# AnamarijaKic/bioinfo1

Hardware: AMD Instinct MI355X
Metric: GCUPS (DP cell updates/s) at 1/2/4/8 GPUs; bit-exact score+CIGAR (higher is better)
Workload: dtype int32 semantics; packed int16 arithmetic where range-proven (fits_int16), else int32; 1 GPU; config 2: 10000 uniform 1000x1000 pairs per GPU, local, scoring 1,-1,-1, CIGAR on; pairs_per_gpu=10000, qlen=1000, tlen=1000, mode=local, cigar=True, cells_per_gpu=10000000000, cells_total=10000000000, parallelism=pairs range-split over 1 GPU(s)

## Files before the change

bioinfo1_amd/csrc/ta_api.hip:

```cpp
#include <hip/hip_runtime.h>
#include <rocprofiler-sdk-roctx/roctx.h>

#include <algorithm>
#include <cstdio>
#include <cstdlib>
#include <cstring>
#include <mutex>
#include <string>
#include <vector>

#include "../../include/team_align_c.h"
#include "ta_context.h"
#include "ta_host_batch.h"
#include "ta_internal.h"
#include "ta_pipeline_internal.h"
#include "ta_plan_driver.h"
#include "ta_planner.h"

using ta_host::fail;

struct TA_PLAN_LOCAL ta_plan : ta::PlanArrays {
    ta_context* ctx = nullptr;
    ta::Plan h;
    void* own_block = nullptr;
    static int exec_chunk(ta_plan* pl, const ta_device_io* io, hipStream_t s, uint32_t c, bool fill, ta::TraceParts trace);
    uint32_t code_layout() const { return h.blk ? (h.ck ? 2u : 1u) : 0u; }
    uint32_t* err_word() const { return h.flexes.empty() && h.duals.empty() && h.single_tasks.empty() ? nullptr : d_err; }
    static const char* err_message(uint32_t err) {
        if (err & ta::kErrWalkCap) return "traceback: a band walk reached its event cap with cost left; results of this plan are invalid";
        return "packed fill: a pass hand-off poll timed out; results of this plan are invalid";
    }
};

namespace {

int check_args(ta_context* ctx, uint32_t n_pairs, const uint32_t* qlen, const uint32_t* tlen, int type) {
    if (!ctx) return TA_ERR_ARG;
    if (n_pairs && (!qlen || !tlen)) return fail(ctx, TA_ERR_ARG, "null argument");
    if (!ta_host::valid_type(type)) return fail(ctx, TA_ERR_BAD_TYPE, ta_status_string(TA_ERR_BAD_TYPE));
    return TA_OK;
}

}

int ta_plan::exec_chunk(ta_plan* pl, const ta_device_io* io, hipStream_t s, uint32_t c, bool fill, ta::TraceParts trace) {
    const ta::Plan& h = pl->h;
    const auto& ch = h.chunks[c];
    ta_context* ctx = pl->ctx;
    if (h.ws_ptr_dwords)
        if (int r = ta_host::grow(ctx, ctx->ws_ptrs, h.ws_ptr_dwords * 4ull)) return r;
    if (h.ws_bnd_words)
        if (int r = ta_host::grow(ctx, ctx->ws_bnd, h.ws_bnd_words * 4ull)) return r;
    if (h.walk_group == 64 && h.want_cigar)
        if (int r = ta_host::grow(ctx, ctx->ws_runs, 4 * (h.slots_bytes + 4))) return r;
    uint32_t* d_ptrs = static_cast<uint32_t*>(ctx->ws_ptrs.p);
    int32_t* d_bnd = static_cast<int32_t*>(ctx->ws_bnd.p);
    if (fill) {
        roctxRangePushA("ta fill");
        if ((ch.fcount || ch.dpasses > 1 || ch.spasses > 1) && ch.bnd_words) TA_HIP(ctx, hipMemsetAsync(d_bnd, 0, ch.bnd_words * 4ull, s));
        ta::FillArgs a{};
        a.order = pl->d_order;
        a.begin = ch.begin;
        a.count = ch.count;
        a.qbytes = reinterpret_cast<const uint8_t*>(io->query_bytes);
        a.qoff = io->query_off;
        a.qlen = pl->d_qlen;
        a.tbytes = reinterpret_cast<const uint8_t*>(io->target_bytes);
        a.toff = io->target_off;
        a.tlen = pl->d_tlen;
        a.match = h.match;
        a.mismatch = h.mismatch;
        a.gap = h.gap;
        a.ptrs = d_ptrs;
        a.ptr_off = pl->d_ptr_off;
        a.bnd = d_bnd;
        a.bnd_off = pl->d_bnd_off;
        a.score = io->score;
        a.target_begin = io->target_begin;
        a.goal_i = pl->d_goal_i;
        a.goal_j = pl->d_goal_j;
        a.fused = h.fused ? 1 : 0;
        a.slots = io->cigar_slots;
        a.slot_off = pl->d_slot_off;
        a.cigar_start = io->cigar_start;
        a.cigar_len = io->cigar_len;
        a.blk = pl->code_layout();
        a.pflag = (h.blk && h.walk_group == 64) ? pl->d_pflag : nullptr;
        if (ch.scount) {
            ta::FillArgs a1 = a;
            a1.order = pl->d_singles;
            a1.begin = ch.sbegin;
            a1.count = ch.scount;
            if (ch.spasses > 1) {
                a1.task_off = pl->d_stask_off;
                a1.tasks64 = pl->d_stasks;
                a1.ticket = pl->d_tickets + 2 * h.chunks.size() + c;
                a1.n_tasks = h.single_task_off[ch.sbegin + ch.scount] - h.single_task_off[ch.sbegin];
                a1.err = pl->d_err;
                a1.pout = pl->d_spout;
                TA_HIP(ctx, hipMemsetAsync(a1.ticket, 0, 4, s));
            }
            if (ch.dcount || ch.fcount) {
                if (int r = ta_host::lazy_stream(ctx, ctx->aux)) return r;
                TA_HIP(ctx, hipEventRecord(ctx->ev_fork, s));
                TA_HIP(ctx, hipStreamWaitEvent(ctx->aux, ctx->ev_fork, 0));
                TA_HIP(ctx, ta::launch_fill(h.type, h.want_cigar, h.wide, a1, ctx->aux));
            } else {
                TA_HIP(ctx, ta::launch_fill(h.type, h.want_cigar, h.wide, a1, s));
            }
        }
        if (ch.dcount || ch.fcount) {
            uint32_t* fb_list = pl->d_fb + 2ull * ch.cbegin;
            uint32_t* fb_count = pl->d_fb + h.n_dual_pairs + c;
            TA_HIP(ctx, hipMemsetAsync(fb_count, 0, 4, s));
            if (ch.dcount) {
                ta::FillArgs d = a;
                d.order = pl->d_duals;
                d.begin = ch.dbegin;
                d.count = ch.dcount;
                d.fb_list = fb_list;
                d.fb_count = fb_count;
                if (ch.dpasses > 1) {
                    d.ticket = pl->d_tickets + h.chunks.size() + c;
                    d.n_tasks = ch.dcount * ch.dpasses;
                    d.epoch = ++ctx->epoch & 0x3FFFFFFu;
                    d.err = pl->d_err;
                    d.pout = pl->d_dpout;
                    d.end_aligned = h.end_aligned ? 1u : 0u;
                    TA_HIP(ctx, hipMemsetAsync(d.ticket, 0, 4, s));
                }
                if (ch.fcount) {
                    if (int r = ta_host::lazy_stream(ctx, ctx->aux2)) return r;
                    TA_HIP(ctx, hipEventRecord(ctx->ev_fork, s));
                    TA_HIP(ctx, hipStreamWaitEvent(ctx->aux2, ctx->ev_fork, 0));
                    TA_HIP(ctx, ta::launch_dual(h.type, h.want_cigar, d, ctx->aux2));
                    TA_HIP(ctx, hipEventRecord(ctx->ev_join2, ctx->aux2));
                } else {
                    TA_HIP(ctx, ta::launch_dual(h.type, h.want_cigar, d, s));
                }
            }
            if (ch.fcount) {
                ta::FillArgs d = a;
                d.order = pl->d_flexes;
                d.begin = ch.fbegin;
                d.count = ch.fcount;
                d.fb_list = fb_list;
                d.fb_count = fb_count;
                d.task_off = pl->d_flex_task_off;
                d.tasks = pl->d_flex_tasks;
                d.ticket = pl->d_tickets + c;
                d.n_tasks = h.flex_task_off[ch.fbegin + ch.fcount] - h.flex_task_off[ch.fbegin];
                d.epoch = ++ctx->epoch & 0x3FFFFFFu;
                d.err = pl->d_err;
                d.pout = pl->d_pout;
                TA_HIP(ctx, hipMemsetAsync(d.ticket, 0, 4, s));
                TA_HIP(ctx, ta::launch_flex(h.type, h.want_cigar, d, s));
            }
            if (ch.dcount && ch.fcount) TA_HIP(ctx, hipStreamWaitEvent(s, ctx->ev_join2, 0));
            ta::FillArgs f = a;
            f.order = fb_list;
            f.begin = 0;
            f.count = 2 * (ch.dcount + ch.fcount);
            f.count_dev = fb_count;
            f.max_blocks = ctx->cu_count;
            TA_HIP(ctx, ta::launch_fill(h.type, h.want_cigar, h.wide, f, s));
        }
        if (ch.scount && (ch.dcount || ch.fcount)) {
            TA_HIP(ctx, hipEventRecord(ctx->ev_join, ctx->aux));
            TA_HIP(ctx, hipStreamWaitEvent(s, ctx->ev_join, 0));
        }
        roctxRangePop();
    }
    if (trace && h.want_cigar && !h.fused) {
        roctxRangePushA("ta traceback");
        ta::TraceArgs t{};
        t.order = pl->d_order;
        t.begin = ch.begin;
        t.count = ch.count;
        t.qlen = pl->d_qlen;
        t.tlen = pl->d_tlen;
        t.ptrs = d_ptrs;
        t.ptr_off = pl->d_ptr_off;
        t.goal_i = pl->d_goal_i;
        t.goal_j = pl->d_goal_j;
        t.slots = io->cigar_slots;
        t.slot_off = pl->d_slot_off;
        t.cigar_start = io->cigar_start;
        t.cigar_len = io->cigar_len;
        t.score = io->score;
        t.qbytes = reinterpret_cast<const uint8_t*>(io->query_bytes);
        t.qoff = io->query_off;
        t.tbytes = reinterpret_cast<const uint8_t*>(io->target_bytes);
        t.toff = io->target_off;
        t.match = h.match;
        t.mismatch = h.mismatch;
        t.gap = h.gap;
        t.blk = pl->code_layout();
        if (h.walk_group == 64) {
            t.pflag = pl->d_pflag;
            t.runs = static_cast<uint32_t*>(ctx->ws_runs.p);
            t.err = pl->d_err;
            t.fb_order = pl->d_fb + 2ull * ch.cbegin;
            t.fb_count = pl->d_fb + h.n_dual_pairs + c;
            TA_HIP(ctx, ta::launch_traceback(h.type, t, s, 64, trace));
        } else {
            TA_HIP(ctx, ta::launch_traceback(h.type, t, s, h.walk_group, trace));
        }
        roctxRangePop();
    }
    return TA_OK;
}

extern "C" {

const char* ta_status_string(int status) {
    switch (status) {
        case TA_OK: return "ok";
        case TA_ERR_BAD_TYPE: return "Unknown AlignmentType provided.";
        case TA_ERR_CIGAR: return "Unknown error in determining cigar string.";
        case TA_ERR_ARG: return "invalid argument";
        case TA_ERR_DEVICE: return "device error";
        case TA_ERR_CAPACITY: return "cigar arena too small";
        case TA_ERR_RANGE: return "affine scoring out of range";
        case TA_ERR_UNSERVED: return "pair outside the single-pair server's limits";
        default: return "unknown status";
    }
}

const char* ta_last_error(const ta_context* ctx) { return ctx ? ctx->last_error.c_str() : ""; }

uint64_t ta_cigar_slot_bytes(uint32_t n, uint32_t m) { return ta::cigar_slot_bytes(n, m); }

int ta_context_create(int device, ta_context** out) {
    if (!out) return TA_ERR_ARG;
    *out = nullptr;
    int count = 0;
    if (hipGetDeviceCount(&count) != hipSuccess || count <= device || device < 0) return TA_ERR_DEVICE;
    hipDeviceProp_t prop;
    if (hipGetDeviceProperties(&prop, device) != hipSuccess) return TA_ERR_DEVICE;
    if (std::strncmp(prop.gcnArchName, "gfx950", 6) != 0) return TA_ERR_DEVICE;
    auto* c = new ta_context();
    c->device = device;
    c->cu_count = (uint32_t)std::max(1, prop.multiProcessorCount);
    if (hipSetDevice(device) != hipSuccess || hipEventCreateWithFlags(&c->ev_join2, hipEventDisableTiming) != hipSuccess ||
        hipEventCreateWithFlags(&c->ev_fork, hipEventDisableTiming) != hipSuccess ||
        hipEventCreateWithFlags(&c->ev_join, hipEventDisableTiming) != hipSuccess ||
        hipEventCreateWithFlags(&c->ev_last, hipEventDisableTiming) != hipSuccess) {
        ta_context_destroy(c);
        return TA_ERR_DEVICE;
    }
    *out = c;
    return TA_OK;
}

void ta_context_release(ta_context* ctx) {
    if (!ctx) return;
    std::lock_guard<std::mutex> lock(ctx->mu);
    (void)hipSetDevice(ctx->device);
    if (ctx->used) (void)hipEventSynchronize(ctx->ev_last);
    for (auto* b : {&ctx->blk, &ctx->out, &ctx->dst, &ctx->ws_ptrs, &ctx->ws_bnd, &ctx->ws_runs}) ta_host::release(*b, false);
    for (auto* b : {&ctx->pin_in, &ctx->pin_out}) ta_host::release(*b, true);
}

int ta_current_device(void) {
    int d = 0;
    return hipGetDevice(&d) == hipSuccess ? d : 0;
}

int ta_device_count(void) {
    int n = 0;
    return hipGetDeviceCount(&n) == hipSuccess ? n : 0;
}

uint64_t ta_context_held_bytes(const ta_context* ctx) {
    if (!ctx) return 0;
    uint64_t n = 0;
    for (const auto* b : {&ctx->ws_ptrs, &ctx->ws_bnd}) n += b->cap;
    return n;
}

void ta_context_destroy(ta_context* ctx) {
    if (!ctx) return;
    ta_context_release(ctx);
    for (hipStream_t s : {ctx->stream, ctx->aux, ctx->aux2})
        if (s) (void)hipStreamDestroy(s);
    for (hipEvent_t e : {ctx->ev_fork, ctx->ev_join, ctx->ev_join2, ctx->ev_last})
        if (e) (void)hipEventDestroy(e);
    delete ctx;
}

void ta_plan_destroy(ta_plan* pl) { ta_host::plan_destroy(pl); }

int ta_plan_create(ta_context* ctx, uint32_t n_pairs, const uint32_t* qlen, const uint32_t* tlen, int type,
                   int match, int mismatch, int gap, int want_cigar, uint64_t budget, uint32_t flags, ta_plan** out) {
    if (!out) return TA_ERR_ARG;
    *out = nullptr;
    if (int r = check_args(ctx, n_pairs, qlen, tlen, type)) return r;
    TA_HIP(ctx, hipSetDevice(ctx->device));
    auto* pl = new ta_plan();
    pl->ctx = ctx;
    ta::build_plan(pl->h, n_pairs, qlen, tlen, type, match, mismatch, gap, want_cigar != 0,
                   budget ? budget : ta_host::default_budget(ctx), flags, 4 * ctx->cu_count);
    return ta_host::plan_create_block(pl, "ta_plan_create: ", out);
}

uint64_t ta_plan_cigar_slots_bytes(const ta_plan* pl) { return pl ? pl->h.slots_bytes : 0; }
uint64_t ta_plan_workspace_bytes(const ta_plan* pl) {
    if (!pl) return 0;
    const ta::Plan& h = pl->h;
    const uint64_t runs = (h.walk_group == 64 && h.want_cigar) ? 4 * (h.slots_bytes + 4) : 0;
    return (h.ws_ptr_dwords + h.ws_bnd_words) * 4ull + runs;
}
uint32_t ta_plan_chunks(const ta_plan* pl) { return pl ? (uint32_t)pl->h.chunks.size() : 0; }
ta_context* ta_plan_context(const ta_plan* pl) { return pl ? pl->ctx : nullptr; }
int ta_context_device(const ta_context* ctx) { return ctx ? ctx->device : -1; }
void ta_context_set_error(ta_context* ctx, const char* message) {
    if (ctx) ctx->last_error = message ? message : "";
}
uint32_t ta_plan_dual_pairs(const ta_plan* pl) { return pl ? pl->h.n_dual_pairs : 0; }
uint32_t ta_plan_flex_pairs(const ta_plan* pl) { return pl ? (uint32_t)pl->h.flexes.size() : 0; }
int ta_plan_fused(const ta_plan* pl) { return pl && pl->h.fused ? 1 : 0; }

int ta_plan_walk(const ta_plan* pl) {
    if (!pl) return -1;
    return pl->h.walk_group | (pl->h.blk ? 0x100 : 0) | (pl->h.ck ? 0x200 : 0);
}

int ta_plan_pair_chunks(const ta_plan* pl, uint32_t* chunk_of_pair) { return ta_host::plan_pair_chunks(pl, chunk_of_pair); }
int ta_plan_execute(ta_plan* pl, const ta_device_io* io, void* stream) { return ta_host::plan_execute(pl, io, stream); }
int ta_plan_execute_fill(ta_plan* pl, const ta_device_io* io, void* stream, uint32_t chunk) {
    return ta_host::plan_execute_chunk(pl, io, stream, chunk, true);
}
int ta_plan_execute_traceback(ta_plan* pl, const ta_device_io* io, void* stream, uint32_t chunk) {
    return ta_host::plan_execute_chunk(pl, io, stream, chunk, false);
}
int ta_plan_execute_walk(ta_plan* pl, const ta_device_io* io, void* stream, uint32_t chunk) {
    return ta_host::plan_execute_chunk(pl, io, stream, chunk, false, ta::kTraceWalk);
}
int ta_plan_execute_format(ta_plan* pl, const ta_device_io* io, void* stream, uint32_t chunk) {
    return ta_host::plan_execute_chunk(pl, io, stream, chunk, false, ta::kTraceFormat);
}
int ta_plan_format_is_split(const ta_plan* pl, uint32_t chunk) {
    if (!pl || chunk >= pl->h.chunks.size() || !pl->h.want_cigar || pl->h.fused) return 0;
    return ta::traceback_has_formatter(pl->h.type, pl->code_layout(), pl->h.walk_group) ? 1 : 0;
}
int ta_plan_check(ta_plan* pl) { return ta_host::plan_check(pl); }
int ta_plan_annotate(ta_plan* pl, const ta_device_io* io, const ta_annotate_io* out, void* stream) {
    return ta_host::plan_annotate(pl, io, out, stream);
}

int ta_compact_cigars(ta_context* ctx, uint32_t n_pairs, const char* cigar_slots, const uint64_t* cigar_start,
                      const uint32_t* cigar_len, const uint64_t* dst_off, char* dst, void* stream) {
    if (!ctx) return TA_ERR_ARG;
    if (!n_pairs) return TA_OK;
    if (!cigar_slots || !cigar_start || !cigar_len || !dst_off || !dst) return fail(ctx, TA_ERR_ARG, "null device pointer");
    TA_HIP(ctx, hipSetDevice(ctx->device));
    ta::CompactArgs ca{n_pairs, cigar_slots, cigar_start, cigar_len, dst_off, dst};
    TA_HIP(ctx, ta::launch_compact(ca, (hipStream_t)stream));
    return TA_OK;
}

int ta_align_batch(ta_context* ctx, uint32_t n_pairs, const char* qb, const uint64_t* qoff, const uint32_t* qlen,
                   const char* tbytes, const uint64_t* toff, const uint32_t* tlen, int type, int match,
                   int mismatch, int gap, int want_cigar, int32_t* score, uint32_t* target_begin, char* arena,
                   uint64_t arena_bytes, uint64_t* cigar_off, uint32_t* cigar_len) {
    return ta_align_batch_flags(ctx, n_pairs, qb, qoff, qlen, tbytes, toff, tlen, type, match, mismatch, gap,
                                want_cigar, score, target_begin, arena, arena_bytes, cigar_off, cigar_len, 0);
}

int ta_align_batch_flags(ta_context* ctx, uint32_t n_pairs, const char* qb, const uint64_t* qoff,
                         const uint32_t* qlen, const char* tbytes, const uint64_t* toff, const uint32_t* tlen,
                         int type, int match, int mismatch, int gap, int want_cigar, int32_t* score,
                         uint32_t* target_begin, char* arena, uint64_t arena_bytes, uint64_t* cigar_off,
                         uint32_t* cigar_len, uint32_t flags) {
    uint64_t qend = 0, tend = 0;
    if (int r = ta_host::check_host_batch(ctx, type, n_pairs, qb, qoff, qlen, tbytes, toff, tlen, want_cigar, arena,
                                          cigar_off, cigar_len, &qend, &tend))
        return r;
    if (n_pairs == 0) return TA_OK;
    std::lock_guard<std::mutex> lock(ctx->mu);
    TA_HIP(ctx, hipSetDevice(ctx->device));
    ta_plan pl;
    pl.ctx = ctx;
    ta::build_plan(pl.h, n_pairs, qlen, tlen, type, match, mismatch, gap, want_cigar != 0,
                   ta_host::batch_budget(ctx, n_pairs, qlen, tlen, want_cigar, 4), flags, 4 * ctx->cu_count);
    return ta_host::host_batch(ctx, pl, n_pairs, qb, qoff, qlen, tbytes, toff, tlen, qend, tend, want_cigar, score,
                               target_begin, arena, arena_bytes, cigar_off, cigar_len);
}

}
```

bioinfo1_amd/csrc/ta_dual.hip:

```cpp
#include "ta_device.h"
#include "ta_packed.h"

namespace ta {
namespace {

#ifdef TA_DUAL_MODE

struct DualOut {
    PassOut o[2];
};

#ifndef TA_DUAL_STAGE
#define TA_DUAL_STAGE 16
#endif
constexpr int kDualStage = TA_DUAL_STAGE;
static_assert(kDualStage == 0 || kDualStage == 8 || kDualStage == 16, "dual BLK staging");
constexpr int kDualStageL = kDualStage ? kDualStage : 16;
#ifndef TA_SWAR
#define TA_SWAR 1
#endif
#ifndef TA_DUAL_CK
#define TA_DUAL_CK 0
#endif
#if defined(TA_DUAL_BLK) && TA_DUAL_CK
constexpr bool kDualCk = true;
#else
constexpr bool kDualCk = false;
#endif
static_assert(!kDualCk || kDualStage != 0, "the checkpoint fill stages each step's bottom row in LDS");

struct DualIo {
    const uint8_t* Q[2];
    const uint8_t* T[2];
    uint32_t* ptrs[2];
    int32_t* B;
    uint64_t* rec_w;
    const uint64_t* rec_r;
    uint32_t tag_w, tag_r;
    uint32_t* err;
    uint32_t* cbuf;
    uint4* lst;
    uint32_t nb;
};

typedef __attribute__((address_space(1))) unsigned long long gu64d;

__device__ __forceinline__ int dual_poll_chunk(const DualIo& io, uint32_t m, uint32_t k, int lane) {
    const uint32_t j = k * 64u + (uint32_t)lane + 1u;
    const gu64d* r = (const gu64d*)(io.rec_r + j);
    int v = 0;
    for (uint32_t spins = 0;; ++spins) {
        bool ok = true;
        if (j <= m) {
            const uint64_t x = __hip_atomic_load(r, __ATOMIC_RELAXED, __HIP_MEMORY_SCOPE_AGENT);
            ok = (uint32_t)(x >> 32) == io.tag_r;
            v = (int)(uint32_t)x;
        }
        if (__builtin_amdgcn_ballot_w64(!ok) == 0) break;
        if (spins > (1u << 22)) {
            if (lane == 0) atomicOr(io.err, 1u);
            break;
        }
        __builtin_amdgcn_s_sleep(2);
    }
    return v;
}

template <int MODE, bool CIGAR, int NV, bool M3, bool CLS, bool BLK = false>
__device__ __forceinline__ DualOut dual_pass(const FillArgs& a, const DualIo& io, uint32_t n, uint32_t m,
                                             uint32_t pass, bool last_pass, int lane, int off = 0) {
    constexpr int R = kRows;
    constexpr bool LOCAL = MODE == kLocal;
    static_assert(!M3 || LOCAL, "three-input maxima: local mode only");
    if constexpr (!M3) off = 0;
    const int ma = a.match, mi = a.mismatch, gap = a.gap;
    const int init = (MODE == kGlobal) ? gap : 0;
    constexpr bool CK = BLK && kDualCk;
    constexpr bool CODES = CIGAR && !CK;
    constexpr bool EQ = M3 && !CODES;
    const int zstep = local_max3_z(ma, EQ);
    const uint32_t KD = rep16(LOCAL ? 16 * (mi - ma) : (mi - ma));
    const uint32_t GL = rep16(LOCAL ? 16 * gap + zstep : 2 * gap - ma);
    const uint32_t GUG = rep16(LOCAL ? 16 * gap - 1 : 0);
    constexpr bool SW = M3 && TA_SWAR;
    uint32_t GLk = swar_k(LOCAL ? 16 * gap + zstep : 2 * gap - ma), GUGk = swar_k(16 * gap - 1);
    asm volatile("" : "+s"(GLk), "+s"(GUGk));
    uint32_t ONE = 0x00010001u;
    asm volatile("" : "+s"(ONE));
    const uint32_t ua = (uint32_t)(16 * ma - 2 + 128), ub = (uint32_t)(16 * mi - 2 + 128);
    const uint32_t T0 = ub * 0x01010101u, TX = ua ^ ub;
    const uint32_t GM = rep16(16 * ma - 2);
    uint32_t KN = swar_k(-128);
    asm volatile("" : "+s"(KN));
    const uint32_t Tmax = pass_steps(m);
    const uint32_t row_base = pass * kPassRows;
    const uint32_t nrows = min((uint32_t)kPassRows, n - row_base);
    const uint32_t nl = (nrows + R - 1) / R;
    const bool has_next = !last_pass;
    constexpr bool UZ = M3;
    const int dl = UZ ? zstep + 16 : 0;
    const uint32_t D2 = rep16(dl);

    uint32_t q2[R], H2[R];
#pragma unroll
    for (int r = 0; r < R; ++r) {
        const uint32_t i0 = row_base + (uint32_t)lane * R + r;
        if constexpr (CLS) q2[r] = i0 < n ? row_selector(io.Q[0][i0], io.Q[1][i0]) : row_selector(0, 0);
        else q2[r] = i0 < n ? ((uint32_t)io.Q[0][i0] | ((uint32_t)io.Q[1][i0] << 16)) : 0u;
        H2[r] = rep16(LOCAL ? off - (int)(i0 + 1) + dl * lane : wmul(i0 + 1, init - gap));
    }
    const uint32_t ia = row_base + (uint32_t)lane * R;
    uint32_t recv = rep16(LOCAL ? off - (int)ia + dl * lane : wmul(ia, init - gap));
    uint32_t tc2 = 0, tA = 0x01010101u, tB = 0x01010101u;
    const uint32_t nv_lane = (uint32_t)lane < nl - 1 ? R : ((uint32_t)lane == nl - 1 ? NV : 0);
    uint32_t Zp = rep16(off + zstep * (0 - lane) - (int)(ia + 1));
    int zu = off - (int)row_base - 1;
    const uint32_t ZS2 = rep16(zstep);
    uint32_t jj = rep16(-lane);
    const uint32_t MAG2 = rep16(ma - gap);
    uint32_t bestK = rep16(-16), bestj = 0;
    uint32_t rowbest = rep16(-32768), rowbest_j = 0;

    constexpr bool LST = CLS && (!BLK || kDualCk);
    uint32_t tcur[2], tnext[2];
    auto tbyte = [&](int h, uint32_t c) -> uint32_t {
        const uint32_t k = c * 64u + (uint32_t)lane;
        return k < m ? (uint32_t)io.T[h][k] : 0u;
    };
    auto table = [&](uint32_t b) -> uint32_t { return EQ ? class_table(b, T0, TX) : mismatch_table(b); };
#pragma unroll
    for (int h = 0; h < 2; ++h) {
        tcur[h] = LST ? tbyte(h, 0) : load_tchunk(io.T[h], m, 0, lane);
        tnext[h] = LST ? tbyte(h, 1) : load_tchunk(io.T[h], m, 1, lane);
    }
    auto top_chunk = [&](uint32_t c) -> int {
        if (pass > 0)
            return (int)pk_sub((uint32_t)(io.rec_r ? dual_poll_chunk(io, m, c, lane) : load_bchunk(io.B, m, c, lane)), D2);
        const int j = (int)(c * 64u + (uint32_t)lane + 1u);
        return (int)rep16(LOCAL ? off + zstep * j - dl : (init - ma + gap) * j);
    };
    int bcur = top_chunk(0), bnext = top_chunk(1);
    if constexpr (LST) {
        __builtin_amdgcn_fence(__ATOMIC_SEQ_CST, "wavefront");
        io.lst[lane] = make_uint4(table(tcur[0]), table(tcur[1]), (uint32_t)bcur, 0u);
        __builtin_amdgcn_fence(__ATOMIC_SEQ_CST, "wavefront");
    }
    const uint32_t steps = m + nl - 1;
    uint32_t* prow0 = CIGAR ? io.ptrs[0] + (BLK ? (uint64_t)pass * io.nb * (kBlkSteps * kWave) : (uint64_t)pass * Tmax * kWave) : nullptr;
    uint32_t* prow1 = CIGAR ? io.ptrs[1] + (BLK ? (uint64_t)pass * io.nb * (kBlkSteps * kWave) : (uint64_t)pass * Tmax * kWave) : nullptr;
    auto ck_flush = [&](uint32_t t, bool full) {
        const uint32_t b = t >> 4;
        uint32_t x[16];
#pragma unroll
        for (int q = 0; q < 16; ++q) x[q] = io.cbuf[q * kWave + lane];
#pragma unroll
        for (int h = 0; h < 2; ++h) {
            const uint32_t sel = h ? 0x07060302u : 0x05040100u;
            uint32_t* dr = (h ? prow1 : prow0) + ((uint64_t)b * kWave + (uint32_t)lane) * 8u;
            __builtin_amdgcn_sched_barrier(0);
#pragma unroll
            for (int q = 0; q < 2; ++q)
                *reinterpret_cast<uint4*>(dr + 4 * q) =
                    make_uint4(__builtin_amdgcn_perm(x[8 * q + 1], x[8 * q], sel), __builtin_amdgcn_perm(x[8 * q + 3], x[8 * q + 2], sel),
                               __builtin_amdgcn_perm(x[8 * q + 5], x[8 * q + 4], sel), __builtin_amdgcn_perm(x[8 * q + 7], x[8 * q + 6], sel));
            if (full) {
                uint32_t* dc = dr + (uint64_t)io.nb * kWave * 8u;
#pragma unroll
                for (int q = 0; q < 2; ++q)
                    *reinterpret_cast<uint4*>(dc + 4 * q) =
                        make_uint4(__builtin_amdgcn_perm(H2[8 * q + 1], H2[8 * q], sel), __builtin_amdgcn_perm(H2[8 * q + 3], H2[8 * q + 2], sel),
                                   __builtin_amdgcn_perm(H2[8 * q + 5], H2[8 * q + 4], sel), __builtin_amdgcn_perm(H2[8 * q + 7], H2[8 * q + 6], sel));
            }
        }
    };
    auto blk_flush = [&](uint32_t t) {
        const uint64_t at = ((uint64_t)(t >> 4) * kWave + (uint32_t)lane) * kBlkSteps + (t & 15u & ~(uint32_t)(kDualStageL - 1));
#pragma unroll
        for (int h = 0; h < 2; ++h) {
            uint32_t* dst = (h ? prow1 : prow0) + at;
            const uint32_t* src = io.cbuf + h * (kDualStageL * kWave) + lane;
#pragma unroll
            for (int q = 0; q < kDualStageL / 4; ++q) {
                __builtin_amdgcn_sched_barrier(0);
                uint4 v;
                v.x = src[(4 * q + 0) * kWave];
                v.y = src[(4 * q + 1) * kWave];
                v.z = src[(4 * q + 2) * kWave];
                v.w = src[(4 * q + 3) * kWave];
                *reinterpret_cast<uint4*>(dst + 4 * q) = v;
            }
        }
    };

    auto reload = [&](uint32_t t) {
        if constexpr (LST) {
            __builtin_amdgcn_fence(__ATOMIC_SEQ_CST, "wavefront");
            io.lst[lane] = make_uint4(table(tnext[0]), table(tnext[1]), (uint32_t)bnext, 0u);
            __builtin_amdgcn_fence(__ATOMIC_SEQ_CST, "wavefront");
#pragma unroll
            for (int h = 0; h < 2; ++h) tnext[h] = tbyte(h, (t >> 6) + 1);
            bnext = top_chunk((t >> 6) + 1);
            return;
        }
        if ((t & 255u) == 0) {
#pragma unroll
            for (int h = 0; h < 2; ++h) {
                tcur[h] = tnext[h];
                tnext[h] = load_tchunk(io.T[h], m, (t >> 8) + 1, lane);
            }
        }
        bcur = bnext;
        bnext = top_chunk((t >> 6) + 1);
    };
    auto step = [&](uint32_t t, auto masked_tag) {
        constexpr bool MASKED = decltype(masked_tag)::value;
        const uint32_t prev = recv;
        if constexpr (LST) {
            const uint4 e = io.lst[t & 63u];
            recv = (uint32_t)wave_shr1((int)e.z, (int)H2[R - 1]);
            tA = (uint32_t)wave_shr1((int)e.x, (int)tA);
            tB = (uint32_t)wave_shr1((int)e.y, (int)tB);
        } else {
            const uint32_t top = (uint32_t)rdlane(bcur, t & 63u);
            const uint32_t sh = (t & 3u) * 8;
            const uint32_t wa = (uint32_t)rdlane((int)tcur[0], (t >> 2) & 63u);
            const uint32_t wb = (uint32_t)rdlane((int)tcur[1], (t >> 2) & 63u);
            const uint32_t newc = ((wa >> sh) & 0xFFu) | (((wb >> sh) & 0xFFu) << 16);
            recv = (uint32_t)wave_shr1((int)top, (int)H2[R - 1]);
            if constexpr (CLS) {
                tA = (uint32_t)wave_shr1((int)table((wa >> sh) & 0xFFu), (int)tA);
                tB = (uint32_t)wave_shr1((int)table((wb >> sh) & 0xFFu), (int)tB);
            } else {
                tc2 = (uint32_t)wave_shr1((int)newc, (int)tc2);
            }
        }
        if constexpr (UZ) recv = pk_add(recv, D2);
        if constexpr (UZ) {
            zu += zstep;
        } else {
            Zp = pk_add(Zp, ZS2);
            if (MODE != kSemi) jj = pk_add(jj, ONE);
        }

        const int j = (int)t - lane + 1;
        const bool active = !MASKED || (((uint32_t)lane < nl) & (j >= 1) & (j <= (int)m));
        uint32_t acc0 = 0, acc1 = 0;
        if (active) {
            auto e_of = [&](int r) {
                if constexpr (CLS) return mismatch_flags(tA, tB, q2[r]);
                else return pk_min_u16(q2[r] ^ tc2, ONE);
            };
            auto diag_of = [&](int r, uint32_t dv) -> uint32_t {
                if constexpr (EQ && CLS) return dv + mismatch_flags(tA, tB, q2[r]) + KN;
                else if constexpr (EQ) return pk_add(pk_mad_i16(e_of(r), KD, dv), GM);
                else return pk_mad_i16(e_of(r), KD, dv);
            };
            uint32_t dnext = diag_of(0, prev);
            uint32_t upv = recv;
            uint32_t Z = Zp;
            uint32_t W[R / 2];
            if constexpr (M3) {
                W[0] = ((uint32_t)zu & 0xFFFFu) * 0x10001u - 0x10000u;
#pragma unroll
                for (int k = 1; k < R / 2; ++k) W[k] = W[0] - 0x20002u * (uint32_t)k;
            }
            static_for<0, R>([&](auto rc) {
                constexpr int r = decltype(rc)::value;
                const uint32_t old = H2[r];
                const uint32_t diag = dnext;
                if constexpr (r + 1 < R) dnext = diag_of(r + 1, old);
                if constexpr (EQ) {
                    const uint32_t lu = pk_max(old, upv);
                    const uint32_t hv = pk_max3_pos_bc<r & 1>(diag, SW ? swar_add(lu, GLk) : pk_add(lu, GL), W[r / 2]);
                    H2[r] = hv;
                    upv = hv;
                    return;
                }
                const uint32_t left = SW ? swar_add(old, GLk) : pk_add(old, GL);
                const uint32_t up = LOCAL ? (SW ? swar_add(upv, GUGk) : pk_add(upv, GUG)) : upv;
                const uint32_t m1 = pk_max(diag, left);
                uint32_t hv;
                if constexpr (M3) hv = pk_max3_pos_bc<r & 1>(m1, up, W[r / 2]);
                else hv = LOCAL ? pk_max(pk_max(m1, up), Z) : pk_max(m1, up);
                if (CODES) {
                    const uint32_t wd = pk_sub_sat(m1, up);
                    const uint32_t wi = pk_sub_sat(diag, left);
                    uint32_t& acc = (r < 8) ? acc0 : acc1;
                    acc = bfi(0x01010101u << (7 - (r & 7)), sign_bytes(wd, wi), acc);
                }
                H2[r] = hv;
                upv = hv;
                if (LOCAL && !M3 && r + 1 < R) Z = pk_sub(Z, ONE);
            });
            if (LOCAL) {
                uint32_t lo, hi_rows = 0;
                if constexpr (M3) {
                    lo = max3_reduce<NV>(H2);
                    if constexpr (NV != R) hi_rows = max3_reduce<R - NV>(H2 + NV);
                } else {
                    lo = tree_max<0, NV>(H2);
                    if constexpr (NV != R) hi_rows = tree_max<NV, R>(H2);
                }
                uint32_t sk = lo;
                if (NV != R) {
                    const uint32_t full = pk_max(lo, hi_rows);
                    sk = ((uint32_t)lane == nl - 1) ? lo : full;
                }
                if constexpr (UZ) {
                    const uint32_t key = pk_sub(sk, ((uint32_t)zu & 0xFFFFu) * 0x10001u);
                    const uint32_t msk = half_mask(pk_sub_sat(bestK, key));
                    bestj = (((t + 1u) * 0x10001u) & msk) | (bestj & ~msk);
                    bestK = pk_max(bestK, key);
                } else {
                    const uint32_t key = pk_sub(sk, Zp);
                    bestj = bfi(half_mask(pk_sub_sat(bestK, key)), jj, bestj);
                    bestK = pk_max(bestK, key);
                }
            }
            if (MODE == kSemi && (NV != R || last_pass)) {
                const uint32_t jl = rep16((int)t + 1 - lane);
                const uint32_t v = pk_mad_i16(jl, MAG2, H2[NV - 1]);
                rowbest_j = bfi(half_mask(pk_sub_sat(rowbest, v)), jl, rowbest_j);
                rowbest = pk_max(rowbest, v);
            }
            if (has_next && (uint32_t)lane == nl - 1) {
                const uint32_t bv = UZ ? pk_sub(H2[R - 1], rep16(dl * lane)) : H2[R - 1];
                if (io.rec_w)
                    __hip_atomic_store((gu64d*)(io.rec_w + j), ((uint64_t)io.tag_w << 32) | bv, __ATOMIC_RELAXED,
                                       __HIP_MEMORY_SCOPE_AGENT);
                else
                    io.B[j] = (int32_t)bv;
            }
        }
        if constexpr (CK) {
            io.cbuf[(t & 15u) * kWave + (uint32_t)lane] = H2[R - 1];
        } else if (CIGAR) {
            const uint32_t cA = __builtin_amdgcn_perm(acc0, acc1, 0x06020400u);
            const uint32_t cB = __builtin_amdgcn_perm(acc0, acc1, 0x07030501u);
            if constexpr (BLK) {
                if constexpr (kDualStage == 0) {
                    const uint32_t off = (uint32_t)blk_index(0, t, (uint32_t)lane, io.nb);
                    prow0[off] = cA;
                    prow1[off] = cB;
                } else {
                    const uint32_t sl = (t & (uint32_t)(kDualStage - 1)) * kWave + (uint32_t)lane;
                    io.cbuf[sl] = cA;
                    io.cbuf[kDualStage * kWave + sl] = cB;
                }
            } else {
                const uint32_t off = (t * kWave + (uint32_t)lane) * 4u;
                *(uint32_t*)((char*)prow0 + off) = cA;
                *(uint32_t*)((char*)prow1 + off) = cB;
            }
        }
    };
    const uint32_t ramp_end = min(nl - 1, steps);
    uint32_t t = 0, next_reload = 64;
    auto run_steps = [&](uint32_t t_end, auto masked_tag) {
        while (t < t_end) {
            if (t == next_reload) {
                reload(t);
                next_reload += 64;
            }
            uint32_t blk = min(t_end, next_reload);
            if constexpr (BLK && kDualStage) blk = min(blk, (t | (uint32_t)(kDualStage - 1)) + 1u);
            for (; t + 1 < blk; t += 2) {
                step(t, masked_tag);
                step(t + 1, masked_tag);
            }
            if (t < blk) step(t++, masked_tag);
            if constexpr (CK) {
                if ((t & 15u) == 0 || t == steps) ck_flush(t - 1, (t & 15u) == 0);
            } else if constexpr (BLK && kDualStage) {
                if ((t & (uint32_t)(kDualStageL - 1)) == 0 || t == steps) blk_flush(t - 1);
            }
        }
    };
    run_steps(ramp_end, std::true_type{});
    run_steps(m, std::false_type{});
    run_steps(steps, std::true_type{});

    DualOut out;
#pragma unroll
    for (int h = 0; h < 2; ++h) {
        PassOut& o = out.o[h];
        o = PassOut{INT_MIN, 0, 0, INT_MIN, 0, 0};
        if (LOCAL) {
            const int K = (h ? hi16(bestK) : lo16(bestK)) + 15;
            const int v = ((uint32_t)lane >= nl || K < 0) ? -1 : (K >> 4);
            const int mx = wave_max(v);
            const int fl = first_lane(v == mx);
            const int Kf = rdlane(K, fl);
            const uint32_t jf = (uint32_t)rdlane((int)(h ? (bestj >> 16) : (bestj & 0xFFFFu)), fl) - (UZ ? (uint32_t)fl : 0u);
            o.h = mx;
            o.i = row_base + (uint32_t)fl * R + (uint32_t)(15 - (Kf & 15)) + 1;
            o.j = jf;
        } else if (MODE == kSemi) {
            int cv = INT_MIN;
            uint32_t cr = 0;
#pragma unroll
            for (int r = 0; r < R; ++r) {
                const int sv = (h ? hi16(H2[r]) : lo16(H2[r])) + gap * (int)(row_base + (uint32_t)lane * R + r + 1);
                if ((uint32_t)r < nv_lane && sv > cv) {
                    cv = sv;
                    cr = r;
                }
            }
            const int mx = wave_max(cv);
            const int fl = first_lane(cv == mx && nv_lane > 0);
            o.h = mx + (ma - gap) * (int)m;
            o.i = row_base + (uint32_t)fl * R + (uint32_t)rdlane((int)cr, fl) + 1;
            o.j = m;
            if (last_pass) {
                const int rb = rdlane(h ? hi16(rowbest) : lo16(rowbest), nl - 1);
                o.row_h = rb == -32768 ? INT_MIN : rb + gap * (int)n;
                o.row_j = (uint32_t)rdlane((int)(h ? (rowbest_j >> 16) : (rowbest_j & 0xFFFFu)), nl - 1);
            }
        } else {
            if (last_pass) {
                int hv[R];
#pragma unroll
                for (int r = 0; r < R; ++r) hv[r] = h ? hi16(H2[r]) : lo16(H2[r]);
                o.corner = rdlane(select_row<R>(hv, nrows - (nl - 1) * R - 1), nl - 1) + (ma - gap) * (int)m + gap * (int)n;
            }
        }
    }
    return out;
}

template <int MODE, bool CIGAR, bool CLS, bool BLK = false>
__device__ __forceinline__ DualOut dual_pass_nv(const FillArgs& a, const DualIo& io, uint32_t n, uint32_t m,
                                                uint32_t pass, bool last_pass, int lane) {
    const uint32_t nrows = min((uint32_t)kPassRows, n - pass * kPassRows);
    const uint32_t nv = nrows - ((nrows + kRows - 1) / kRows - 1) * kRows;
    if constexpr (MODE == kLocal) {
        constexpr bool eq = !CIGAR || (BLK && kDualCk);
        const int off = local_max3_offset(n, m, a.match, a.mismatch, a.gap, eq);
        if (off >= 0) {
            if (nv == kRows)
                return dual_pass<MODE, CIGAR, kRows, true, CLS, BLK>(a, io, n, m, pass, last_pass, lane, off);
#define TA_NV_CASE(k) \
    case k: return dual_pass<MODE, CIGAR, k, true, CLS, BLK>(a, io, n, m, pass, last_pass, lane, off);
            switch (nv) {
                TA_NV_CASE(1) TA_NV_CASE(2) TA_NV_CASE(3) TA_NV_CASE(4) TA_NV_CASE(5) TA_NV_CASE(6) TA_NV_CASE(7)
                TA_NV_CASE(8) TA_NV_CASE(9) TA_NV_CASE(10) TA_NV_CASE(11) TA_NV_CASE(12) TA_NV_CASE(13) TA_NV_CASE(14)
                default: TA_NV_CASE(15)
            }
#undef TA_NV_CASE
        }
    }
    if (MODE == kGlobal || nv == kRows)
        return dual_pass<MODE, CIGAR, kRows, false, CLS, BLK>(a, io, n, m, pass, last_pass, lane);
#define TA_NV_CASE(k) \
    case k: return dual_pass<MODE, CIGAR, k, false, CLS, BLK>(a, io, n, m, pass, last_pass, lane);
    switch (nv) {
        TA_NV_CASE(1) TA_NV_CASE(2) TA_NV_CASE(3) TA_NV_CASE(4) TA_NV_CASE(5) TA_NV_CASE(6) TA_NV_CASE(7)
        TA_NV_CASE(8) TA_NV_CASE(9) TA_NV_CASE(10) TA_NV_CASE(11) TA_NV_CASE(12) TA_NV_CASE(13) TA_NV_CASE(14)
        default: TA_NV_CASE(15)
    }
#undef TA_NV_CASE
}

#ifndef TA_DUAL_WAVES
#define TA_DUAL_WAVES 5
#endif
constexpr uint32_t kDualSkip = 0xFFFFFFFFu;

template <int MODE, bool CIGAR, bool BLK = false>
__device__ __forceinline__ void dual_fill_body(const FillArgs& a) {
    const int lane = threadIdx.x & 63;
    constexpr int kStageDw = kDualCk ? 16 * kWave : 2 * kDualStage * kWave;
    __shared__ uint32_t cbuf_all[(BLK && kDualStage) ? kWavesPerBlock * kStageDw : 1];
    __shared__ uint4 lst_all[(BLK && !kDualCk) ? 1 : kWavesPerBlock * 64];
    uint32_t widx, p_only = 0;
    const bool pipe = a.ticket != nullptr;
    if (pipe) {
        uint32_t tk = 0;
        if (lane == 0) tk = atomicAdd(a.ticket, 1u);
        tk = (uint32_t)__builtin_amdgcn_readfirstlane((int)tk);
        if (tk >= a.n_tasks) return;
        p_only = tk / a.count;
        widx = tk - p_only * a.count;
    } else {
        widx = wave_id();
        if (widx >= a.count) return;
    }
    uint32_t p[2];
    p[0] = a.order[2 * (a.begin + widx)];
    p[1] = a.order[2 * (a.begin + widx) + 1];
    const uint32_t n = a.qlen[p[0]], m = a.tlen[p[0]];
    const uint32_t passes = n_passes(n);
    if (pipe && a.end_aligned) {
        const uint32_t shift = a.n_tasks / a.count - passes;
        if (p_only < shift) return;
        p_only -= shift;
    }
    if (pipe && p_only >= passes) return;
    PassOut* po = pipe ? static_cast<PassOut*>(a.pout) + 2ull * ((uint64_t)p_only * a.count + widx) : nullptr;
    DualIo io;
    io.rec_w = nullptr;
    io.rec_r = nullptr;
    io.tag_w = io.tag_r = 0;
    io.err = a.err;
    io.cbuf = cbuf_all + ((BLK && kDualStage) ? (threadIdx.x >> 6) * kStageDw : 0);
    io.lst = lst_all + (threadIdx.x >> 6) * 64;
    io.nb = blk_count(m);
    bool dash = false, qother = false;
#pragma unroll
    for (int h = 0; h < 2; ++h) {
        io.Q[h] = a.qbytes + a.qoff[p[h]];
        io.T[h] = a.tbytes + a.toff[p[h]];
        io.ptrs[h] = CIGAR ? a.ptrs + a.ptr_off[p[h]] : nullptr;
        for (uint32_t k = (uint32_t)lane; k < m; k += 64) dash |= io.T[h][k] == '-';
        for (uint32_t k = (uint32_t)lane; k < n; k += 64) {
            const uint32_t c = io.Q[h][k];
            dash |= c == '-';
            qother |= !is_acgt(c);
        }
    }
    const bool cls = __ballot(qother) == 0;
    const bool any_dash = __ballot(dash) != 0;
    if (a.pflag && lane == 0 && (!pipe || p_only == 0)) {
        a.pflag[p[0]] = any_dash ? 1 : 0;
        a.pflag[p[1]] = any_dash ? 1 : 0;
    }
    if (any_dash) {
        if (lane == 0) {
            if (!pipe || p_only == 0) {
                const uint32_t k = (p[1] != p[0]) ? 2u : 1u;
                const uint32_t at = atomicAdd(a.fb_count, k);
                a.fb_list[at] = p[0];
                if (k == 2) a.fb_list[at + 1] = p[1];
            }
            if (pipe) {
                po[0].i = kDualSkip;
                po[1].i = kDualSkip;
            }
        }
        return;
    }
    io.B = (passes > 1) ? a.bnd + a.bnd_off[p[0]] : nullptr;
    if (pipe) {
        uint64_t* rec = reinterpret_cast<uint64_t*>(io.B);
        const uint64_t rb = (uint64_t)m + 1;
        io.rec_w = (p_only + 1 == passes) ? nullptr : rec + (p_only & 1u) * rb;
        io.rec_r = p_only ? rec + ((p_only - 1u) & 1u) * rb : nullptr;
        io.tag_w = a.epoch * 64u + p_only + 1u;
        io.tag_r = a.epoch * 64u + p_only;
        const bool last_pass = p_only + 1 == passes;
        const DualOut o = cls ? dual_pass_nv<MODE, CIGAR, true, BLK>(a, io, n, m, p_only, last_pass, lane)
                              : dual_pass_nv<MODE, CIGAR, false, BLK>(a, io, n, m, p_only, last_pass, lane);
        if (lane == 0) {
            po[0] = o.o[0];
            po[1] = o.o[1];
        }
        return;
    }
    int best_h[2], corner[2] = {0, 0};
    uint32_t best_i[2], best_j[2];
#pragma unroll
    for (int h = 0; h < 2; ++h) {
        best_h[h] = (MODE == kSemi) ? 0 : INT_MIN;
        best_i[h] = 0;
        best_j[h] = (MODE == kSemi) ? m : 0;
    }
    for (uint32_t pass = 0; pass < passes; ++pass) {
        const bool last_pass = pass + 1 == passes;
        const DualOut o = cls ? dual_pass_nv<MODE, CIGAR, true, BLK>(a, io, n, m, pass, last_pass, lane)
                              : dual_pass_nv<MODE, CIGAR, false, BLK>(a, io, n, m, pass, last_pass, lane);
#pragma unroll
        for (int h = 0; h < 2; ++h) {
            if (MODE != kGlobal && o.o[h].h > best_h[h]) {
                best_h[h] = o.o[h].h;
                best_i[h] = o.o[h].i;
                best_j[h] = o.o[h].j;
            }
            if (MODE == kSemi && last_pass && o.o[h].row_h > best_h[h]) {
                best_h[h] = o.o[h].row_h;
                best_i[h] = n;
                best_j[h] = o.o[h].row_j;
            }
            if (MODE == kGlobal && last_pass) corner[h] = o.o[h].corner;
        }
        if (!last_pass) __builtin_amdgcn_fence(__ATOMIC_SEQ_CST, "workgroup");
    }
    if (CIGAR && a.fused) {
        __builtin_amdgcn_fence(__ATOMIC_RELEASE, "workgroup");
        __builtin_amdgcn_fence(__ATOMIC_ACQUIRE, "workgroup");
    }
#pragma unroll
    for (int h = 0; h < 2; ++h) {
        const uint32_t gi = (MODE == kGlobal) ? n : best_i[h], gj = (MODE == kGlobal) ? m : best_j[h];
        if (CIGAR && a.fused) {
            uint64_t st;
            uint32_t len;
            const WalkSeq seq{io.Q[h], io.T[h], best_h[h], a.match, a.mismatch, a.gap};
            traceback_pair<MODE>(io.ptrs[h], n, m, gi, gj, a.slots + a.slot_off[p[h]], cigar_slot_bytes(n, m), lane,
                                 &st, &len, seq);
            if (lane == 0) {
                a.cigar_start[p[h]] = a.slot_off[p[h]] + st;
                a.cigar_len[p[h]] = len;
            }
        }
        if (lane == 0) {
            a.score[p[h]] = (MODE == kGlobal) ? corner[h] : best_h[h];
            a.target_begin[p[h]] = (MODE == kLocal) ? best_j[h] + 1 : 0;
            a.goal_i[p[h]] = gi;
            a.goal_j[p[h]] = gj;
        }
    }
}

template <int MODE, bool CIGAR, bool BLK = false>
__global__ __launch_bounds__(kBlock) __attribute__((amdgpu_waves_per_eu(TA_DUAL_WAVES))) void dual_fill_kernel(FillArgs a) {
    dual_fill_body<MODE, CIGAR, BLK>(a);
}
#if defined(TA_DUAL_BLK) && TA_DUAL_CK
template <int MODE>
__global__ __launch_bounds__(kBlock) __attribute__((amdgpu_waves_per_eu(TA_DUAL_WAVES))) void dual_fill_ck_kernel(FillArgs a) {
    dual_fill_body<MODE, true, true>(a);
}
#endif

inline dim3 dual_grid(uint32_t waves) { return dim3((waves + kWavesPerBlock - 1) / kWavesPerBlock); }

template <int MODE>
__global__ void dual_combine_kernel(FillArgs a) {
    const uint32_t w = blockIdx.x * blockDim.x + threadIdx.x;
    if (w >= a.count) return;
    const PassOut* po = static_cast<const PassOut*>(a.pout);
    if (po[2ull * w].i == kDualSkip) return;
    const uint32_t n = a.qlen[a.order[2 * (a.begin + w)]], m = a.tlen[a.order[2 * (a.begin + w)]];
    const uint32_t passes = n_passes(n);
#pragma unroll
    for (int h = 0; h < 2; ++h) {
        const uint32_t p = a.order[2 * (a.begin + w) + h];
        int best_h = (MODE == kSemi) ? 0 : INT_MIN, corner = 0;
        uint32_t best_i = 0, best_j = (MODE == kSemi) ? m : 0;
        for (uint32_t k = 0; k < passes; ++k) {
            const PassOut& o = po[2ull * ((uint64_t)k * a.count + w) + h];
            if (MODE != kGlobal && o.h > best_h) {
                best_h = o.h;
                best_i = o.i;
                best_j = o.j;
            }
            if (MODE == kSemi && k + 1 == passes && o.row_h > best_h) {
                best_h = o.row_h;
                best_i = n;
                best_j = o.row_j;
            }
            if (MODE == kGlobal && k + 1 == passes) corner = o.corner;
        }
        if (h == 1 && p == a.order[2 * (a.begin + w)]) break;
        a.score[p] = (MODE == kGlobal) ? corner : best_h;
        a.target_begin[p] = (MODE == kLocal) ? best_j + 1 : 0;
        a.goal_i[p] = (MODE == kGlobal) ? n : best_i;
        a.goal_j[p] = (MODE == kGlobal) ? m : best_j;
    }
}

#endif
}

#ifdef TA_DUAL_MODE
#if defined(TA_DUAL_BLK) && TA_DUAL_CK
template <>
hipError_t launch_dual_ck<TA_DUAL_MODE>(const FillArgs& a, hipStream_t s) {
#elif defined(TA_DUAL_BLK)
hipError_t launch_dual_blk(const FillArgs& a, hipStream_t s) {
#else
template <>
hipError_t launch_dual_mode<TA_DUAL_MODE, (TA_DUAL_CIGAR != 0)>(const FillArgs& a, hipStream_t s) {
#endif
    if (!a.count) return hipSuccess;
#if defined(TA_DUAL_BLK) && TA_DUAL_CK
    hipLaunchKernelGGL(dual_fill_ck_kernel<TA_DUAL_MODE>, dual_grid(a.ticket ? a.n_tasks : a.count), dim3(kBlock), 0, s,
                       a);
#elif defined(TA_DUAL_BLK)
    hipLaunchKernelGGL((dual_fill_kernel<TA_DUAL_MODE, true, true>), dual_grid(a.ticket ? a.n_tasks : a.count),
                       dim3(kBlock), 0, s, a);
#else
#if TA_DUAL_CIGAR
    if (a.blk == 2) return launch_dual_ck<TA_DUAL_MODE>(a, s);
#endif
#if TA_DUAL_MODE == 1 && TA_DUAL_CIGAR
    if (a.blk) return launch_dual_blk(a, s);
#endif
    hipLaunchKernelGGL((dual_fill_kernel<TA_DUAL_MODE, TA_DUAL_CIGAR != 0>), dual_grid(a.ticket ? a.n_tasks : a.count),
                       dim3(kBlock), 0, s, a);
#endif
    if (a.ticket)
        hipLaunchKernelGGL(dual_combine_kernel<TA_DUAL_MODE>, dim3((a.count + 255) / 256), dim3(256), 0, s, a);
    return hipGetLastError();
}
#endif

}
```

bioinfo1_amd/csrc/ta_internal.h:

```cpp
#pragma once

#include <hip/hip_runtime.h>
#include <stdint.h>

#include "../../include/team_align_c.h"
#include "ta_layout.h"

namespace ta {

enum Code : uint32_t { kCodeM = 0, kCodeI = 1, kCodeD = 2, kCodeStop = 3 };
constexpr int kDPlane = 16;

struct FillArgs {
    const uint32_t* order;
    uint32_t begin, count;
    const uint8_t* qbytes;
    const uint64_t* qoff;
    const uint32_t* qlen;
    const uint8_t* tbytes;
    const uint64_t* toff;
    const uint32_t* tlen;
    int match, mismatch, gap;
    uint32_t* ptrs;
    const uint64_t* ptr_off;
    int32_t* bnd;
    const uint64_t* bnd_off;
    int32_t* score;
    uint32_t* target_begin;
    uint32_t* goal_i;
    uint32_t* goal_j;
    int fused;
    char* slots;
    const uint64_t* slot_off;
    uint64_t* cigar_start;
    uint32_t* cigar_len;
    uint32_t* fb_list;
    uint32_t* fb_count;
    const uint32_t* count_dev;
    uint32_t max_blocks;
    const uint32_t* task_off;
    const uint32_t* tasks;
    uint32_t* ticket;
    uint32_t n_tasks;
    uint32_t epoch;
    uint32_t* err;
    void* pout;
    const uint64_t* tasks64;
    uint32_t end_aligned;
    uint32_t blk;
    uint8_t* pflag;
};

constexpr uint32_t kErrPassPoll = 1u;
constexpr uint32_t kErrWalkCap = 2u;
__host__ __device__ inline uint64_t band_runs_off(uint64_t slot_off) { return (slot_off + 3u) & ~(uint64_t)3u; }

struct TraceArgs {
    const uint32_t* order;
    uint32_t begin, count;
    const uint32_t* qlen;
    const uint32_t* tlen;
    const uint32_t* ptrs;
    const uint64_t* ptr_off;
    const uint32_t* goal_i;
    const uint32_t* goal_j;
    char* slots;
    const uint64_t* slot_off;
    uint64_t* cigar_start;
    uint32_t* cigar_len;
    const int32_t* score;
    const uint8_t* qbytes;
    const uint64_t* qoff;
    const uint8_t* tbytes;
    const uint64_t* toff;
    int match, mismatch, gap;
    uint32_t blk;
    const uint8_t* pflag;
    uint32_t* runs;
    uint32_t* err;
    const uint32_t* fb_order;
    const uint32_t* fb_count;
};

struct CompactArgs {
    uint32_t n_pairs;
    const char* slots;
    const uint64_t* cigar_start;
    const uint32_t* cigar_len;
    const uint64_t* dst_off;
    char* dst;
};

struct AnnotateArgs {
    uint32_t n_pairs;
    int mode;
    const uint32_t* qlen;
    const uint32_t* tlen;
    const uint32_t* goal_i;
    const uint32_t* goal_j;
    const uint64_t* slot_off;
    const uint8_t* qbytes;
    const uint64_t* qoff;
    const uint8_t* tbytes;
    const uint64_t* toff;
    const char* slots;
    const uint64_t* cigar_start;
    const uint32_t* cigar_len;
    ta_pair_info* info;
    char* eqx_slots;
    uint64_t* eqx_start;
    uint32_t* eqx_len;
};

struct BandCertifyArgs {
    uint32_t n_pairs;
    int mode, match, mismatch, gap_open, gap_extend;
    const uint32_t* qlen;
    const uint32_t* tlen;
    const uint32_t* band;
    const uint8_t* qbytes;
    const uint64_t* qoff;
    const uint8_t* tbytes;
    const uint64_t* toff;
    const int32_t* score;
    uint8_t* exact;
    uint32_t* band_needed;
};

constexpr uint32_t kSrvQMax = 4096;
constexpr uint32_t kSrvTMax = 16384;
constexpr uint64_t kSrvStride = 65536;
constexpr uint64_t kSrvQOff = 128, kSrvTOff = kSrvQOff + kSrvQMax, kSrvCOff = kSrvTOff + kSrvTMax;
static_assert(kSrvCOff + 2 * (kSrvQMax + kSrvTMax) + 2 <= kSrvStride, "server slot too small");

struct ServeHdr {
    uint32_t seq;
    uint32_t n, m;
    int32_t match, mismatch, gap;
    uint32_t want_cigar;
    uint32_t pad0[9];
    uint32_t done;
    int32_t score;
    uint32_t target_begin, cigar_len, status;
    uint32_t pad1[11];
};
static_assert(sizeof(ServeHdr) == kSrvQOff, "ServeHdr layout");

struct ServeCtl {
    uint32_t stop;
    uint32_t heartbeat;
    uint32_t pad[14];
};

struct ServeArgs {
    char* host;
    const ServeCtl* ctl;
    FillArgs fa;
    uint64_t hb_timeout;
};

hipError_t launch_fill(int mode, bool cigar, bool wide, const FillArgs& a, hipStream_t s);
template <int MODE, bool CIGAR>
hipError_t launch_fill_mode(bool wide, const FillArgs& a, hipStream_t s);
enum TraceParts : int { kTraceWalk = 1, kTraceFormat = 2, kTraceAll = 3 };
bool traceback_has_formatter(int mode, uint32_t blk, int group);
hipError_t launch_traceback(int mode, const TraceArgs& a, hipStream_t s, int group, int parts = kTraceAll);
hipError_t launch_dual(int mode, bool cigar, const FillArgs& a, hipStream_t s);
template <int MODE, bool CIGAR>
hipError_t launch_dual_mode(const FillArgs& a, hipStream_t s);
hipError_t launch_dual_blk(const FillArgs& a, hipStream_t s);
template <int MODE>
hipError_t launch_dual_ck(const FillArgs& a, hipStream_t s);
hipError_t launch_walk_ck(int mode, const TraceArgs& a, hipStream_t s);
template <int MODE>
hipError_t launch_flex_ck(const FillArgs& a, hipStream_t s);
hipError_t launch_flex(int mode, bool cigar, const FillArgs& a, hipStream_t s);
template <int MODE, bool CIGAR>
hipError_t launch_flex_mode(const FillArgs& a, hipStream_t s);
hipError_t launch_compact(const CompactArgs& a, hipStream_t s);
hipError_t launch_annotate(const AnnotateArgs& a, hipStream_t s);
hipError_t launch_band_certify(const BandCertifyArgs& a, hipStream_t s);
template <int MODE>
hipError_t launch_serve_mode(const ServeArgs& a, uint32_t slots, hipStream_t s);
hipError_t launch_serve(int mode, const ServeArgs& a, uint32_t slots, hipStream_t s);

}
```

Before: 8518 GCUPS.

## Track best block per checkpoint flush and resolve goal column in a follow-up kernel

In the checkpointed local dual fill, the per-step best-column tracking (a packed compare and select every DP step) is dropped. Instead, the best block index is recorded once per checkpoint flush. A new small kernel then recomputes that one 16x16 block from the stored checkpoints to find the exact goal column. This removes per-cell bookkeeping from the hot loop. In exchange it adds an extra launch and a verification path that flags an error if the block does not reproduce the score.

```diff
diff --git a/bioinfo1_amd/csrc/ta_api.hip b/bioinfo1_amd/csrc/ta_api.hip
--- a/bioinfo1_amd/csrc/ta_api.hip
+++ b/bioinfo1_amd/csrc/ta_api.hip
@@ -28,6 +28,7 @@
     uint32_t* err_word() const { return h.flexes.empty() && h.duals.empty() && h.single_tasks.empty() ? nullptr : d_err; }
     static const char* err_message(uint32_t err) {
         if (err & ta::kErrWalkCap) return "traceback: a band walk reached its event cap with cost left; results of this plan are invalid";
+        if (err & ta::kErrGoalResolve) return "checkpoint fill: a goal's block does not hold its score; results of this plan are invalid";
         return "packed fill: a pass hand-off poll timed out; results of this plan are invalid";
     }
 };
@@ -120,11 +121,11 @@
                 d.count = ch.dcount;
                 d.fb_list = fb_list;
                 d.fb_count = fb_count;
+                d.err = pl->d_err;
                 if (ch.dpasses > 1) {
                     d.ticket = pl->d_tickets + h.chunks.size() + c;
                     d.n_tasks = ch.dcount * ch.dpasses;
                     d.epoch = ++ctx->epoch & 0x3FFFFFFu;
-                    d.err = pl->d_err;
                     d.pout = pl->d_dpout;
                     d.end_aligned = h.end_aligned ? 1u : 0u;
                     TA_HIP(ctx, hipMemsetAsync(d.ticket, 0, 4, s));
diff --git a/bioinfo1_amd/csrc/ta_dual.hip b/bioinfo1_amd/csrc/ta_dual.hip
--- a/bioinfo1_amd/csrc/ta_dual.hip
+++ b/bioinfo1_amd/csrc/ta_dual.hip
@@ -1,4 +1,5 @@
 #include "ta_device.h"
+#include "ta_goal_resolve.h"
 #include "ta_packed.h"
 
 namespace ta {
@@ -119,6 +120,7 @@
     uint32_t jj = rep16(-lane);
     const uint32_t MAG2 = rep16(ma - gap);
     uint32_t bestK = rep16(-16), bestj = 0;
+    uint32_t bestKp = rep16(-16), bestb = 0;
     uint32_t rowbest = rep16(-32768), rowbest_j = 0;
 
     constexpr bool LST = CLS && (!BLK || kDualCk);
@@ -150,6 +152,11 @@
     uint32_t* prow1 = CIGAR ? io.ptrs[1] + (BLK ? (uint64_t)pass * io.nb * (kBlkSteps * kWave) : (uint64_t)pass * Tmax * kWave) : nullptr;
     auto ck_flush = [&](uint32_t t, bool full) {
         const uint32_t b = t >> 4;
+        if constexpr (LOCAL && UZ) {
+            const uint32_t msk = half_mask(pk_sub_sat(bestKp, bestK));
+            bestb = ((b * 0x10001u) & msk) | (bestb & ~msk);
+            bestKp = bestK;
+        }
         uint32_t x[16];
 #pragma unroll
         for (int q = 0; q < 16; ++q) x[q] = io.cbuf[q * kWave + lane];
@@ -308,8 +315,10 @@
                 }
                 if constexpr (UZ) {
                     const uint32_t key = pk_sub(sk, ((uint32_t)zu & 0xFFFFu) * 0x10001u);
-                    const uint32_t msk = half_mask(pk_sub_sat(bestK, key));
-                    bestj = (((t + 1u) * 0x10001u) & msk) | (bestj & ~msk);
+                    if constexpr (!CK) {
+                        const uint32_t msk = half_mask(pk_sub_sat(bestK, key));
+                        bestj = (((t + 1u) * 0x10001u) & msk) | (bestj & ~msk);
+                    }
                     bestK = pk_max(bestK, key);
                 } else {
                     const uint32_t key = pk_sub(sk, Zp);
@@ -391,7 +400,11 @@
             const int mx = wave_max(v);
             const int fl = first_lane(v == mx);
             const int Kf = rdlane(K, fl);
-            const uint32_t jf = (uint32_t)rdlane((int)(h ? (bestj >> 16) : (bestj & 0xFFFFu)), fl) - (UZ ? (uint32_t)fl : 0u);
+            uint32_t jf;
+            if constexpr (CK && UZ)
+                jf = (uint32_t)rdlane((int)(h ? (bestb >> 16) : (bestb & 0xFFFFu)), fl);
+            else
+                jf = (uint32_t)rdlane((int)(h ? (bestj >> 16) : (bestj & 0xFFFFu)), fl) - (UZ ? (uint32_t)fl : 0u);
             o.h = mx;
             o.i = row_base + (uint32_t)fl * R + (uint32_t)(15 - (Kf & 15)) + 1;
             o.j = jf;
@@ -659,6 +672,28 @@
     }
 }
 
+#if defined(TA_DUAL_BLK) && TA_DUAL_CK && TA_DUAL_MODE == 1
+__global__ void ck_goal_resolve_kernel(FillArgs a) {
+    const uint32_t w = blockIdx.x * blockDim.x + threadIdx.x;
+    if (w >= 2u * a.count) return;
+    const uint32_t p0 = a.order[2 * (a.begin + (w >> 1))], p = a.order[2 * (a.begin + (w >> 1)) + (w & 1u)];
+    if ((w & 1u) && p == p0) return;
+    if (a.pflag && a.pflag[p] == 1) return;
+    const uint32_t n = a.qlen[p], m = a.tlen[p];
+    const int off = local_max3_offset(n, m, a.match, a.mismatch, a.gap, true);
+    if (off < 0 || n == 0 || m == 0) return;
+    const uint32_t j = ck_goal_resolve(reinterpret_cast<const uint16_t*>(a.ptrs + a.ptr_off[p]), a.qbytes + a.qoff[p],
+                                       a.tbytes + a.toff[p], n, m, a.match, a.mismatch, a.gap, off, a.score[p],
+                                       a.goal_i[p], a.goal_j[p]);
+    if (!j) {
+        if (a.err) atomicOr(a.err, kErrGoalResolve);
+        return;
+    }
+    a.goal_j[p] = j;
+    a.target_begin[p] = j + 1;
+}
+#endif
+
 #endif
 }
 
@@ -691,6 +726,9 @@
 #endif
     if (a.ticket)
         hipLaunchKernelGGL(dual_combine_kernel<TA_DUAL_MODE>, dim3((a.count + 255) / 256), dim3(256), 0, s, a);
+#if defined(TA_DUAL_BLK) && TA_DUAL_CK && TA_DUAL_MODE == 1
+    hipLaunchKernelGGL(ck_goal_resolve_kernel, dim3((2 * a.count + 255) / 256), dim3(256), 0, s, a);
+#endif
     return hipGetLastError();
 }
 #endif
diff --git a/bioinfo1_amd/csrc/ta_goal_resolve.h b/bioinfo1_amd/csrc/ta_goal_resolve.h
--- /dev/null
+++ b/bioinfo1_amd/csrc/ta_goal_resolve.h
@@ -0,0 +1,68 @@
+#pragma once
+
+#include <stdint.h>
+
+#include "ta_layout.h"
+
+#if defined(__clang__)
+#define TA_UNROLL _Pragma("unroll")
+#else
+#define TA_UNROLL
+#endif
+
+namespace ta {
+
+TA_HD inline uint32_t ck_goal_resolve(const uint16_t* P, const uint8_t* Q, const uint8_t* T, uint32_t n, uint32_t m,
+                                      int ma, int mi, int gap, int off, int score, uint32_t gi, uint32_t b) {
+    const uint32_t nb = blk_count(m);
+    if (gi < 1 || gi > n || b >= nb || score < 0) return 0;
+    const int z = local_max3_z(ma, true), dl = z + 16;
+    const uint32_t g = (gi - 1) >> 4, l = g & 63u, pass = g >> 6;
+    const int r = (int)((gi - 1) & 15u);
+    const int jlo = 16 * (int)b - (int)l + 1, jhi = jlo + 15;
+    const int c_first = jlo > 1 ? jlo : 1, c_last = jhi < (int)m ? jhi : (int)m;
+    if (c_first > c_last) return 0;
+    const int cl = c_first - 1;
+    const uint32_t lu = (g - 1) & 63u, pu = (g - 1) >> 6;
+    int tv[kBlkSteps + 1];
+    int tb[kBlkSteps];
+    TA_UNROLL
+    for (int x = 0; x <= kBlkSteps; ++x) {
+        const int j = cl + x;
+        tv[x] = 0;
+        if (g > 0 && j >= 1 && j <= c_last)
+            tv[x] = ck_decode(P[ck_row_index(pu, (uint32_t)j + lu - 1u, lu, nb)], off, z, dl, 16 * (int)g, j, (int)lu);
+        if (x < kBlkSteps) tb[x] = j + 1 <= c_last ? (int)T[j] : -1;
+    }
+    int h[kRows], qb[kRows];
+    TA_UNROLL
+    for (int k = 0; k < kRows; ++k) {
+        h[k] = 0;
+        qb[k] = -2;
+        if (k <= r) qb[k] = Q[16u * g + (uint32_t)k];
+        if (k <= r && cl > 0)
+            h[k] = ck_decode(P[ck_col_index(pass, b - 1u, l, nb, (uint32_t)k)], off, z, dl, 16 * (int)g + k + 1, cl, (int)l);
+    }
+    TA_UNROLL
+    for (int x = 0; x < kBlkSteps; ++x) {
+        int up = tv[x + 1], dg = tv[x], hr = 0;
+        TA_UNROLL
+        for (int k = 0; k < kRows; ++k) {
+            const int old = h[k];
+            int v = dg + (qb[k] == tb[x] ? ma : mi);
+            v = v > up + gap ? v : up + gap;
+            v = v > old + gap ? v : old + gap;
+            v = v > 0 ? v : 0;
+            h[k] = v;
+            hr = k == r ? v : hr;
+            up = v;
+            dg = old;
+        }
+        if (cl + x + 1 <= c_last && hr == score) return (uint32_t)(cl + x + 1);
+    }
+    return 0;
+}
+
+#undef TA_UNROLL
+
+}
diff --git a/bioinfo1_amd/csrc/ta_internal.h b/bioinfo1_amd/csrc/ta_internal.h
--- a/bioinfo1_amd/csrc/ta_internal.h
+++ b/bioinfo1_amd/csrc/ta_internal.h
@@ -53,6 +53,7 @@
 
 constexpr uint32_t kErrPassPoll = 1u;
 constexpr uint32_t kErrWalkCap = 2u;
+constexpr uint32_t kErrGoalResolve = 4u;
 __host__ __device__ inline uint64_t band_runs_off(uint64_t slot_off) { return (slot_off + 3u) & ~(uint64_t)3u; }
 
 struct TraceArgs {
```

Result: slower. 8285 GCUPS (-2.7%).
